# UPM-ROB-Lab/Vision-basedSensor

Measured on AMD Instinct MI355X. Metric: frames/sec (track->3D) at 1280x1024, 169 markers, higher is better.
Workload: dtype u8+f64; 1 GPU; BASELINE config 3/4: 4096 synthetic 1280x1024 gray uint8 frames per GPU (13x13 dots, seeded jitter+noise), resident in HBM; fused track->3D table + last-seen displacement; frames_per_gpu=4096, internal_batch=1536, pass_streams=2, markers=169, channels=1, world_size=1, backend=none (single process), distinct_devices=1, tracked_observations=692224, xyz_solved=692224, ncc_ambiguous_pixels=205, ncc_exact_pixels=11244250, ncc_counter_frames=839680

## Files before the change

vision-basedsensor_amd/csrc/k_ncc_mfma.hip:

```cpp
#include <algorithm>
#include <cstddef>
#include <cstring>
#include <type_traits>

#include "ncc_common.h"

typedef _Float16 h8 __attribute__((ext_vector_type(8)));
typedef _Float16 h4 __attribute__((ext_vector_type(4)));
typedef float f4 __attribute__((ext_vector_type(4)));
typedef float f2 __attribute__((ext_vector_type(2)));
typedef int i4 __attribute__((ext_vector_type(4)));
typedef __attribute__((address_space(1))) u8 gl_u8;
typedef __attribute__((address_space(1))) unsigned short gl_u16;

template <int L> struct NccLit;
template <> struct NccLit<80> { static constexpr float kc = 163.84f, ks2 = 547.2815085234848f, K1 = 3502601.654550303f; };
template <> struct NccLit<33> { static constexpr float kc = 962.8797061524332f, ks2 = 6956.564407359948f, K1 = 7575698.639614983f; };

struct NccKArgs {
    const u64* bits; const double* rx; const double* ry; const uint4* wfrag; const double* tab; const float2* rowf;
    u64* mbits; u8* mask_u8; u32* fstat; u64* tot;
    int H, W, WW, tiles_per_seg, dbg_arg; float rel_arg;
    NccConst nc;
};
typedef __attribute__((address_space(4))) const NccKArgs NccKArgsC;
__device__ __forceinline__ NccKArgsC* ncc_kargs() {
    NccKArgsC* p = (NccKArgsC*)__builtin_amdgcn_kernarg_segment_ptr();
    asm volatile("" : "+s"(p));
    return p;
}

template <int L, int LO, bool U8OUT>
__global__ __launch_bounds__(256, 4) void k_ncc_mfma(const u64* __restrict__ bits, const double* __restrict__ rx,
                                                     const double* __restrict__ ry, const uint4* __restrict__ wfrag,
                                                     const double* __restrict__ tab, const float2* __restrict__ rowf,
                                                     u64* __restrict__ mbits, u8* __restrict__ mask_u8,
                                                     u32* __restrict__ fstat, u64* __restrict__ tot, int H, int W, int WW,
                                                     int tiles_per_seg,
                                                     int dbg_arg, float rel_arg, NccConst nc) {
#ifdef VBS_DEBUG_KNOBS
    const int dbg = dbg_arg & (NCC_TRIM_BIT - 1);
#else
    constexpr int dbg = 0;
#endif
    constexpr int HI = L - 1 + LO;
    constexpr int NT = (16 + L - 1 + 15) / 16;
    constexpr int NKS = (16 * NT + 31) / 32;
    constexpr int NK8 = (16 * NT + 63) / 64;
    constexpr int RING = 16 * NT;
    constexpr int RSTR = RING + 8;
    constexpr int CSTR = RING + 16;
    constexpr int ECAP = 2 * NT + 2;
    __shared__ struct __align__(16) {
        uint4 lut[256];
        _Float16 ring[4][2][16 * RSTR];
        u8 ringc[4][16 * CSTR];
        u32 elist[4][ECAP][10];
    } sm;
    const int tid = threadIdx.x, lane = tid & 63;
    const int wave = __builtin_amdgcn_readfirstlane(tid >> 6);
    const int g = lane >> 4, q = lane & 15;
    const int n = blockIdx.z;
    const int tilesY = (H + 15) / 16;
    const int tile0 = blockIdx.y * tiles_per_seg;
    int ntiles = min(tiles_per_seg, tilesY - tile0);
    if (ntiles <= 0) return;
    int Y0 = tile0 * 16;
    const int xw = blockIdx.x * 64 + 16 * wave;
    const u64* fbits = bits + (int64_t)n * H * WW;
    {
        u32 w[4];
#pragma unroll
        for (int d = 0; d < 4; ++d) w[d] = (((u32)tid >> (2 * d)) & 1u ? 0x3C00u : 0u) | (((u32)tid >> (2 * d + 1)) & 1u ? 0x3C000000u : 0u);
        sm.lut[tid] = make_uint4(w[0], w[1], w[2], w[3]);
    }
    if (dbg_arg & NCC_TRIM_BIT) {
        const int seg_y0 = Y0, seg_y1 = min(Y0 + 16 * ntiles, H);
        const int r0 = max(Y0 + LO, 0), r1 = min(Y0 + 16 * ntiles - 1 + HI, H - 1);
        const int pws = xw + LO, pb0 = pws >> 3;
        const bool pwide = (pb0 >= 0) && ((pb0 & ~3) + 16 <= 8 * WW);
        constexpr int NB = 16 + L - 1;
        int first = 0x7FFFFFFF, last = -1;
        for (int base = r0; base <= r1; base += 256) {
            u64 w0[4], w1[4];
#pragma unroll
            for (int k = 0; k < 4; ++k) {
                const int row = min(base + 64 * k + lane, r1);
                if (pwide) {
                    const uint4 rr = *reinterpret_cast<const uint4*>(reinterpret_cast<const u8*>(fbits) + (pb0 & ~3) + (int64_t)row * (8 * WW));
                    const u64 lo64 = (u64)rr.x | ((u64)rr.y << 32), hi64 = (u64)rr.z | ((u64)rr.w << 32);
                    const int sh = 8 * (pb0 & 3);
                    w0[k] = sh ? (lo64 >> sh) | (hi64 << (64 - sh)) : lo64;
                    w1[k] = hi64 >> sh;
                } else {
                    const u64* prow = fbits + (int64_t)row * WW;
                    w0[k] = load_bits(prow, WW, pws);
                    w1[k] = NB > 64 ? load_bits(prow, WW, pws + 64) : 0ull;
                }
            }
#pragma unroll
            for (int k = 0; k < 4; ++k) {
                const u64 v0 = NB >= 64 ? w0[k] : w0[k] & ((1ull << (NB & 63)) - 1ull);
                const u64 v1 = NB > 64 ? w1[k] & ((1ull << ((NB - 64) & 63)) - 1ull) : 0ull;
                const u64 occ = __ballot((v0 | v1) != 0ull);
                if (occ) {
                    first = min(first, min(base + 64 * k + (int)__builtin_ctzll(occ), r1));
                    last = max(last, min(base + 64 * k + 63 - (int)__builtin_clzll(occ), r1));
                }
            }
        }
        int ta = tile0;
        if (last >= 0) {
            const int tb = min(Y0 + 16 * ntiles - 1, last - LO) >> 4;
            ta = max(Y0, first - HI) >> 4;
            ntiles = tb - ta + 1;
        } else {
            ntiles = 0;
        }
        Y0 = 16 * __builtin_amdgcn_readfirstlane(ta);
        ntiles = __builtin_amdgcn_readfirstlane(ntiles);
        u8* zb = reinterpret_cast<u8*>(reinterpret_cast<unsigned short*>(mbits) + ((int64_t)n * H * WW + blockIdx.x) * 4 + wave);
        for (int y = seg_y0 + lane; y < seg_y1; y += 64)
            if (y < Y0 || y >= Y0 + 16 * ntiles) *reinterpret_cast<unsigned short*>(zb + (int64_t)y * (8 * WW)) = 0;
        if (U8OUT) {
            for (int y = seg_y0 + g; y < seg_y1; y += 4)
                if ((y < Y0 || y >= Y0 + 16 * ntiles) && xw + q < W) mask_u8[((int64_t)n * H + y) * W + xw + q] = 0;
        }
    }
    const int nsteps = ntiles > 0 ? ntiles + NT - 1 : 0;
    h8 whi[NKS], wlo[NKS], one[NKS];
    i4 one8[NK8];
    if (nsteps) {
        for (int i = lane; i < 2 * 16 * RSTR / 8; i += 64) reinterpret_cast<uint4*>(&sm.ring[wave][0][0])[i] = make_uint4(0, 0, 0, 0);
        for (int i = lane; i < 16 * CSTR / 16; i += 64) reinterpret_cast<uint4*>(&sm.ringc[wave][0])[i] = make_uint4(0, 0, 0, 0);
#pragma unroll
        for (int s = 0; s < NKS; ++s) {
            uint4 a = wfrag[(0 * NKS + s) * 64 + lane], b = wfrag[(1 * NKS + s) * 64 + lane], c = wfrag[(2 * NKS + s) * 64 + lane];
            whi[s] = __builtin_bit_cast(h8, a);
            wlo[s] = __builtin_bit_cast(h8, b);
            one[s] = __builtin_bit_cast(h8, c);
        }
#pragma unroll
        for (int s = 0; s < NK8; ++s) {
            const uint4 a = wfrag[(3 * NKS + s) * 64 + lane];
            one8[s] = i4{(int)a.x, (int)a.y, (int)a.z, (int)a.w};
        }
    }
    __builtin_amdgcn_s_waitcnt(0x0F70);
    __syncthreads();

    const double mu = (double)(255ull * (u64)fstat[n * 8 + 0]) / (double)((int64_t)H * W);
    const double full_t = ry[min(max(-LO, 0), H - 1)] * rx[min(max(-LO, 0), W - 1)];
    auto uni = [](float v) { float o; asm("s_nop 4\n\tv_readfirstlane_b32 %0, %1\n\ts_nop 4" : "=s"(o) : "v"(v)); return o; };
    const float kc = uni((float)(nc.tbar * (NCC_WSCALE * NCC_WSCALE)));
    const float th0 = (float)ncc_theta(0.0, nc.l2, full_t, mu, nc);
    bool lit_ok;
    {
        const double ksd = sqrt(nc.thr2 * nc.T2) / (double)L * (NCC_WSCALE * NCC_WSCALE);
        const double k0d = mu * (full_t - nc.l2 * nc.tbar) / 255.0 * (NCC_WSCALE * NCC_WSCALE);
        lit_ok = fabs(nc.tbar * (NCC_WSCALE * NCC_WSCALE) - (double)NccLit<L>::kc) <= 2e-7 * (double)NccLit<L>::kc &&
                 fabs(ksd * ksd - (double)NccLit<L>::ks2) <= 2e-7 * (double)NccLit<L>::ks2 && fabs(k0d) < 1e-4;
    }
    const bool th0pos = __builtin_amdgcn_readfirstlane((th0 > 0.0f && lit_ok) ? 1 : 0) != 0;
    const bool xin = (xw + LO >= 0) && (xw + 15 + HI <= W - 1);
#ifdef VBS_DEBUG_KNOBS
    const int plain_lo = dbg == 10 ? -0x40000000 : (th0pos && xin && dbg != 11) ? -LO : 0x7FFFFFFF, plain_hi = dbg == 10 ? 0x40000000 : H - 1 - 15 - HI;
#else
    const int plain_lo = (th0pos && xin) ? -LO : 0x7FFFFFFF, plain_hi = H - 1 - 15 - HI;
#endif
    const int valid_hi = (xw + 15 < W) ? H - 16 : -1;
    const float muf = uni((float)mu), tbarf = uni((float)nc.tbar), ktf = uni((float)(nc.tbar * 255.0)), il2f = uni((float)nc.inv_l2);
    const float krf = uni((float)(nc.thr2 * nc.T2));
    const float mukf = uni((float)(mu / 255.0 * (NCC_WSCALE * NCC_WSCALE)));
    const int xq = min(xw + q, W - 1);
    const float nxf = (float)(min(xq + HI, W - 1) - max(xq + LO, 0) + 1), rxf = (float)rx[xq];
    const float nnc = (float)L * nxf, stc = (float)ry[min(max(-LO, 0), H - 1)] * rxf, dd0c = stc - nnc * tbarf;
    _Float16* const ringw = &sm.ring[wave][0][q * RSTR];
    _Float16* const wr = ringw + 4 * g;
    const _Float16* const rd = ringw + 8 * g;
    const _Float16* const rdw = rd - (g >= 2 ? RING : 0);
    u8* const cw = &sm.ringc[wave][q * CSTR] + 4 * g;
    const u8* const cbase = &sm.ringc[wave][q * CSTR];
    constexpr int LOFS = 16 * RSTR;
    u32 amb = 0, nexact = 0;
    unsigned short* mb16 = reinterpret_cast<unsigned short*>(mbits) + ((int64_t)n * H * WW + blockIdx.x) * 4 + wave;
    const int wstart = xw + LO;
    static_assert((LO & 7) == 0, "the window must start on a byte of the row");
    const int rowbytes = 8 * WW, b0 = wstart >> 3;
    int wide_i = __builtin_amdgcn_readfirstlane(((b0 >= 0) && ((b0 & ~3) + 16 <= rowbytes)) ? 1 : 0);
    asm volatile("" : "+s"(wide_i));
#define wide (wide_i != 0)
    uint4 nraw = make_uint4(0, 0, 0, 0);
    const u8* fby = reinterpret_cast<const u8*>(fbits) + (b0 & ~3);
    const u32 lofs = (u32)(q * rowbytes);
    const u32 psel = 0x0C0C0C00u | (u32)((b0 & 3) + g);
    auto load_rows = [&](int t) {
        const int ytile = Y0 + LO + 16 * t;
        if (wide) {
            const gl_u8* pg;
            if (ytile >= 0 && ytile + 15 < H) {
                const u8* pb = fby + (int64_t)ytile * rowbytes;
                asm volatile("" : "+s"(pb));
                u32 lo_ = lofs;
                asm volatile("" : "+v"(lo_));
                pg = (const gl_u8*)pb + lo_;
            } else {
                pg = (const gl_u8*)fby + (u32)__mul24(min(max(ytile + q, 0), H - 1), rowbytes);
            }
            typedef u32 u32x4 __attribute__((ext_vector_type(4)));
            typedef __attribute__((address_space(1))) const u32x4 gl_u4;
            const u32x4 rr = *(gl_u4*)pg;
            nraw = make_uint4(rr.x, rr.y, rr.z, rr.w);
        } else {
            const u64* row = fbits + (int64_t)min(max(ytile + q, 0), H - 1) * WW;
            int ws = __builtin_amdgcn_readfirstlane(wstart);
            asm volatile("" : "+s"(ws));
            const u64 w0 = load_bits(row, WW, ws), w1 = NKS > 2 ? load_bits(row, WW, ws + 64) : 0ull;
            const u32 dw[4] = {(u32)w0, (u32)(w0 >> 32), (u32)w1, (u32)(w1 >> 32)};
            const u32 sh = 8 * (b0 & 3);
            nraw = make_uint4(dw[0] << sh, sh ? __builtin_amdgcn_alignbit(dw[1], dw[0], 32 - sh) : dw[1],
                              sh ? __builtin_amdgcn_alignbit(dw[2], dw[1], 32 - sh) : dw[2],
                              sh ? __builtin_amdgcn_alignbit(dw[3], dw[2], 32 - sh) : dw[3]);
        }
    };
    int ecnt = 0;
    constexpr int NO_TILE = 0x7FFFFFFF;
    u32 pend_x = 0;
    int pend_yo = NO_TILE;
    const u32 off_lo = (u32)((8 * (lane & 1) + ((lane >> 1) & 3)) * rowbytes), off_hi = off_lo + (u32)(4 * rowbytes);
    auto flush_pending = [&]() {
        if (pend_yo != NO_TILE) {
            u8* base = reinterpret_cast<u8*>(mb16) + (int64_t)pend_yo * rowbytes;
            asm volatile("" : "+s"(base));
            gl_u8* bg = (gl_u8*)base;
            u32 ol_ = off_lo, oh_ = off_hi;
            asm volatile("" : "+v"(ol_), "+v"(oh_));
            if (pend_yo <= H - 16) {
                if (lane < 8) {
                    *(gl_u16*)(bg + ol_) = (unsigned short)pend_x;
                    *(gl_u16*)(bg + oh_) = (unsigned short)(pend_x >> 16);
                }
            } else {
                const int rl = pend_yo + 8 * (lane & 1) + ((lane >> 1) & 3);
                if (lane < 8 && rl < H) *(gl_u16*)(bg + ol_) = (unsigned short)pend_x;
                if (lane < 8 && rl + 4 < H) *(gl_u16*)(bg + oh_) = (unsigned short)(pend_x >> 16);
            }
        }
        pend_yo = NO_TILE;
    };
    auto drain = [&]() {
        __builtin_amdgcn_s_waitcnt(0x0F70);
        constexpr bool RELOAD = L < 64;
        const double *d_tab, *d_rx, *d_ry; u64* d_mbits; u8* d_mask_u8; int d_H, d_W, d_WW;
        double d_nc_tbar, d_nc_inv_l2, d_nc_thr2, d_nc_T2, d_mu; const u64* d_fbits;
        if constexpr (RELOAD) {
            NccKArgsC* ka = ncc_kargs();
            d_tab = ka->tab; d_rx = ka->rx; d_ry = ka->ry; d_mbits = ka->mbits; d_mask_u8 = ka->mask_u8;
            d_H = ka->H; d_W = ka->W; d_WW = ka->WW;
            d_nc_tbar = ka->nc.tbar; d_nc_inv_l2 = ka->nc.inv_l2; d_nc_thr2 = ka->nc.thr2; d_nc_T2 = ka->nc.T2;
            d_mu = (double)(255ull * (u64)ka->fstat[n * 8 + 0]) / (double)((int64_t)d_H * d_W);
            d_fbits = ka->bits + (int64_t)n * d_H * d_WW;
        } else {
            d_tab = tab; d_rx = rx; d_ry = ry; d_mbits = mbits; d_mask_u8 = mask_u8; d_H = H; d_W = W; d_WW = WW;
            d_nc_tbar = nc.tbar; d_nc_inv_l2 = nc.inv_l2; d_nc_thr2 = nc.thr2; d_nc_T2 = nc.T2; d_mu = mu; d_fbits = fbits;
        }
        const double* cgd = d_tab + VBS_NCC_MAXL;
        u32* mb32 = reinterpret_cast<u32*>(d_mbits) + (int64_t)n * d_H * d_WW * 2;
        for (int e = 0; e < ecnt; ++e) {
            const int yo = (int)__builtin_amdgcn_readfirstlane((int)sm.elist[wave][e][0]);
#pragma unroll 1
            for (int r = 0; r < 4; ++r) {
                u64 ur = (u64)(u32)__builtin_amdgcn_readfirstlane((int)sm.elist[wave][e][2 + 2 * r]) |
                         ((u64)(u32)__builtin_amdgcn_readfirstlane((int)sm.elist[wave][e][3 + 2 * r]) << 32);
                while (ur) {
                    const int l = __ffsll((long long)ur) - 1;
                    ur &= ur - 1ull;
                    const int y = yo + 4 * (l >> 4) + r, xe = xw + (l & 15);
                    double hv[(L + 63) / 64];
                    u32 cnt = 0;
#pragma unroll
                    for (int k = 0; k < (L + 63) / 64; ++k) {
                        const int i = lane + 64 * k, yy = y + LO + i;
                        hv[k] = (i < L && yy >= 0 && yy < d_H) ? ncc_row_exact<L, LO>(d_fbits + (int64_t)yy * d_WW, d_WW, xe, cgd, &cnt) : 0.0;
                    }
#pragma unroll
                    for (int off = 32; off >= 1; off >>= 1) cnt += (u32)__shfl_xor((int)cnt, off);
                    double Ge = 0.0;
#pragma unroll
                    for (int k = 0; k < (L + 63) / 64; ++k) {
                        const u32 hl = (u32)__double_as_longlong(hv[k]), hh = (u32)((u64)__double_as_longlong(hv[k]) >> 32);
#pragma unroll 8
                        for (int i = 64 * k; i < min(L, 64 * k + 64); ++i) {
                            const u64 hb = (u64)(u32)__builtin_amdgcn_readlane((int)hl, i - 64 * k) |
                                           ((u64)(u32)__builtin_amdgcn_readlane((int)hh, i - 64 * k) << 32);
                            Ge = __builtin_fma(d_tab[i], __longlong_as_double((long long)hb), Ge);
                        }
                    }
                    int ny = min(y + HI, d_H - 1) - max(y + LO, 0) + 1;
                    int nx = min(xe + HI, d_W - 1) - max(xe + LO, 0) + 1;
                    double nn = (double)(ny * nx), sum_t = d_ry[y] * d_rx[xe];
                    double sum_I = 255.0 * (double)cnt;
                    double rest = -d_nc_tbar * sum_I - d_mu * (sum_t - nn * d_nc_tbar);
                    double s1 = sum_I - nn * d_mu;
                    double s2 = 255.0 * sum_I - 2.0 * d_mu * sum_I + nn * d_mu * d_mu;
                    double var = s2 - s1 * s1 * d_nc_inv_l2;
                    double rhs = d_nc_thr2 * var * d_nc_T2;
                    double num = 255.0 * Ge + rest;
                    const int flags = __builtin_amdgcn_readfirstlane((var > 0.0 ? 1 : 0) | ((var > 0.0 && num > 0.0 && num * num > rhs) ? 2 : 0) |
                                                                     ((var > 1e-6 && num > 0.0 && fabs(num * num - rhs) <= 1e-9 * rhs) ? 4 : 0));
                    if ((flags & 2) && lane == 0) {
                        atomicOr(&mb32[(u32)__mul24(y, 2 * d_WW) + (u32)(xe >> 5)], 1u << (xe & 31));
                        if (U8OUT) d_mask_u8[((int64_t)n * d_H + y) * d_W + xe] = 1;
                    }
                    if (flags & 1) { nexact++; if (flags & 4) amb++; }
                }
            }
        }
        ecnt = 0;
    };
    h8 a_op[NKS];
    auto fetch_ops = [&](int tt) {
        u32 by[NKS];
        const u32 rw[5] = {nraw.x, nraw.y, nraw.z, nraw.w, 0u};
#pragma unroll
        for (int s = 0; s < NKS; ++s) by[s] = __builtin_amdgcn_perm(rw[s + 1], rw[s], psel);
#pragma unroll
        for (int s = 0; s < NKS; ++s) asm volatile("" : "+v"(by[s]) :: "memory");
        load_rows(tt + 1);
        flush_pending();
        const int ytile = Y0 + LO + 16 * tt;
        if (ytile < 0 || ytile + 15 >= H) {
            const bool rowin = (ytile + q >= 0) && (ytile + q < H);
#pragma unroll
            for (int s = 0; s < NKS; ++s) by[s] = rowin ? by[s] : 0u;
        }
#pragma unroll
        for (int s = 0; s < NKS; ++s) a_op[s] = __builtin_bit_cast(h8, sm.lut[by[s]]);
    };
    if (nsteps) {
        load_rows(0);
        fetch_ops(0);
    }
    for (int t0 = 0; t0 < nsteps; t0 += NT) {
#pragma unroll
        for (int u = 0; u < NT; ++u) {
            const int t = t0 + u;
            if (t >= nsteps) break;
            constexpr int dummy_nt = NT;
            const int B = (u + 1) % dummy_nt;
            constexpr int NKE = (RING - 16) / 32;
            constexpr int NK8E = (RING - 16) / 64;
            f4 G = {0, 0, 0, 0};
            i4 C = {0, 0, 0, 0};
            auto vert_f16 = [&](int s) {
                const int r0 = (16 * B + 32 * s) % RING;
                const _Float16* p = (r0 + 32 <= RING ? rd : rdw) + r0;
                const h8 bh = *reinterpret_cast<const h8*>(p);
                const h8 bl = *reinterpret_cast<const h8*>(p + LOFS);
                G = __builtin_amdgcn_mfma_f32_16x16x32_f16(whi[s], bh, G, 0, 0, 0);
                G = __builtin_amdgcn_mfma_f32_16x16x32_f16(whi[s], bl, G, 0, 0, 0);
                G = __builtin_amdgcn_mfma_f32_16x16x32_f16(wlo[s], bh, G, 0, 0, 0);
            };
            auto vert_i8 = [&](int s) {
                const int gi = min(4 * s + g, NT - 1);
                const int slot = B + gi - (gi >= NT - B ? NT : 0);
                const i4 bc = *reinterpret_cast<const i4*>(cbase + 16 * slot);
                C = __builtin_amdgcn_mfma_i32_16x16x64_i8(one8[s], bc, C, 0, 0, 0);
            };
            const bool vert = !(t < NT - 1 || dbg == 3);
            f4 ah = {0, 0, 0, 0}, ac = {0, 0, 0, 0};
            if (vert) {
#pragma unroll
                for (int s = 0; s < NKS; ++s) {
                    ah = __builtin_amdgcn_mfma_f32_16x16x32_f16(a_op[s], whi[s], ah, 0, 0, 0);
                    if (s < NKE) vert_f16(s);
                    ah = __builtin_amdgcn_mfma_f32_16x16x32_f16(a_op[s], wlo[s], ah, 0, 0, 0);
                    if (s < NK8E) vert_i8(s);
                    ac = __builtin_amdgcn_mfma_f32_16x16x32_f16(a_op[s], one[s], ac, 0, 0, 0);
                }
#pragma unroll
                for (int s = NKS; s < NKE; ++s) vert_f16(s);
            } else {
#pragma unroll
                for (int s = 0; s < NKS; ++s) {
                    ah = __builtin_amdgcn_mfma_f32_16x16x32_f16(a_op[s], whi[s], ah, 0, 0, 0);
                    ah = __builtin_amdgcn_mfma_f32_16x16x32_f16(a_op[s], wlo[s], ah, 0, 0, 0);
                    ac = __builtin_amdgcn_mfma_f32_16x16x32_f16(a_op[s], one[s], ac, 0, 0, 0);
                }
            }
            fetch_ops(t + 1);
            {
                h4 vh, vl;
#pragma unroll
                for (int r = 0; r < 4; ++r) {
                    const float hi_f = __uint_as_float(__float_as_uint(ah[r]) & 0xFFFFE000u);
                    vh[r] = (_Float16)hi_f;
                    vl[r] = (_Float16)(ah[r] - hi_f);
                }
                u32 vc = 0;
#pragma unroll
                for (int r = 0; r < 4; ++r) vc = __builtin_amdgcn_cvt_pk_u8_f32(ac[r], r, vc);
                *reinterpret_cast<h4*>(wr + 16 * u) = vh;
                *reinterpret_cast<h4*>(wr + LOFS + 16 * u) = vl;
                *reinterpret_cast<u32*>(cw + 16 * u) = vc;
            }
            if (!vert) continue;
            const int yo = Y0 + 16 * (t - (NT - 1));
#pragma unroll
            for (int s = NKE; s < NKS; ++s) vert_f16(s);
#pragma unroll
            for (int s = NK8E; s < NK8; ++s) vert_i8(s);
#ifdef VBS_DEBUG_KNOBS
            if (dbg == 8 && mask_u8) {
#pragma unroll
                for (int r = 0; r < 4; ++r) {
                    const int y = yo + 4 * g + r, x = xw + q;
                    if (y < H && x < W) mask_u8[((int64_t)n * H + y) * W + x] = (u8)C[r];
                }
                continue;
            }
#endif
            if (dbg == 2) { asm volatile("" :: "v"(G[0]), "v"(G[1]), "v"(G[2]), "v"(G[3]), "v"(C[0]), "v"(C[1]), "v"(C[2]), "v"(C[3])); continue; }
            const int x = xw + q;
            float cf[4];
#pragma unroll
            for (int r = 0; r < 4; ++r) cf[r] = (float)C[r];
            u64 pw[4] = {0, 0, 0, 0}, uw[4] = {0, 0, 0, 0};
            if (yo >= plain_lo && yo <= plain_hi) {
                const float rel = rel_arg;
                float uu[4], uhi[4];
#pragma unroll
                for (int r = 0; r < 4; ++r) {
                    uu[r] = __builtin_fmaf(cf[r], -NccLit<L>::kc, G[r]);
                    uhi[r] = __builtin_fmaf(G[r], rel, uu[r]);
                }
                const float umax = fmaxf(fmaxf(uhi[0], uhi[1]), fmaxf(uhi[2], uhi[3]));
                if (__ballot(umax >= 0.0f) || dbg == 12) {
#pragma unroll
                    for (int r = 0; r < 4; ++r) {
                        const float ulo = __builtin_fmaf(G[r], -rel, uu[r]);
                        const float a = __builtin_fmaf(cf[r], -NccLit<L>::ks2, NccLit<L>::K1) * cf[r];
                        pw[r] = __ballot(ulo * fabsf(ulo) > a);
                        uw[r] = ~(pw[r] | __ballot(uhi[r] * fabsf(uhi[r]) <= a));
                    }
                }
            } else {
                float nnv[4], stv[4], dd0[4], uhi[4];
                if (yo + LO >= 0 && yo <= plain_hi) {
#pragma unroll
                    for (int r = 0; r < 4; ++r) { nnv[r] = nnc; stv[r] = stc; dd0[r] = dd0c; }
                } else {
#pragma unroll
                    for (int r = 0; r < 4; ++r) {
                        const float2 rf = rowf[min(yo + 4 * g + r, H - 1)];
                        nnv[r] = rf.x * nxf;
                        stv[r] = rf.y * rxf;
                        dd0[r] = stv[r] - nnv[r] * tbarf;
                    }
                }
#pragma unroll
                for (int r = 0; r < 4; ++r) {
                    const float kcc = kc * cf[r];
                    const float mrg = __builtin_fmaf(1e-3f, G[r] + kcc, __builtin_fmaf(1e-5f * mukf, stv[r], 2.0f));
                    uhi[r] = (G[r] - kcc) - mukf * dd0[r] + mrg;
                }
                if (__ballot(fmaxf(fmaxf(uhi[0], uhi[1]), fmaxf(uhi[2], uhi[3])) >= 0.0f)) {
#pragma unroll
                    for (int r = 0; r < 4; ++r) {
                        const float cfr = cf[r];
                        const float nn = nnv[r], a0 = 1.0f - nn * il2f;
                        const float rest = -(ktf * cfr) - muf * dd0[r];
                        const float var = 65025.0f * cfr * (1.0f - cfr * il2f) + a0 * muf * (nn * muf - 510.0f * cfr);
                        const float t1 = (__builtin_amdgcn_sqrtf(fmaxf(krf * var, 0.0f)) - rest) * (float)(NCC_WSCALE * NCC_WSCALE / 255.0);
                        const float t0v = ((dd0[r] > -1e-4f) | (dd0[r] * dd0[r] < 0.5f * krf * a0 * nn)) ? (float)NCC_NEVER : 0.0f;
                        const float th = cfr == 0.0f ? t0v : t1;
                        const float m = __builtin_fmaf(fabsf(th), 1e-3f, 2.0f), d = G[r] - th;
                        pw[r] = __ballot(d > m);
                        uw[r] = ~(pw[r] | __ballot(d < -m));
                    }
                }
            }
            if (yo > valid_hi) {
#pragma unroll
                for (int r = 0; r < 4; ++r) {
                    const u64 v = __ballot((yo + 4 * g + r < H) && (x < W));
                    pw[r] &= v; uw[r] &= v;
                }
            }
#ifdef VBS_DEBUG_KNOBS
            if (dbg == 9 && mask_u8) {
#pragma unroll
                for (int r = 0; r < 4; ++r) {
                    const int y = yo + 4 * g + r;
                    if (y < H && x < W) mask_u8[((int64_t)n * H + y) * W + x] = (u8)(((pw[r] >> lane) & 1ull) | (((uw[r] >> lane) & 1ull) << 1));
                }
                continue;
            }
#endif
            if (uw[0] | uw[1] | uw[2] | uw[3]) {
                if (lane == 0) {
                    u32* e = &sm.elist[wave][ecnt][0];
                    e[0] = (u32)yo;
#pragma unroll
                    for (int r = 0; r < 4; ++r) { e[2 + 2 * r] = (u32)uw[r]; e[3 + 2 * r] = (u32)(uw[r] >> 32); }
                }
                ecnt++;
            }
            if (U8OUT) {
#pragma unroll
                for (int r = 0; r < 4; ++r) {
                    const int y = yo + 4 * g + r;
                    if (y < H && x < W) mask_u8[((int64_t)n * H + y) * W + x] = (u8)((pw[r] >> lane) & 1ull);
                }
            }
            if (dbg == 1) { asm volatile("" :: "s"(pw[0]), "s"(pw[1]), "s"(pw[2]), "s"(pw[3])); continue; }
            {
                u32 xv = 0;
#pragma unroll
                for (int r = 0; r < 4; ++r) {
                    asm("v_writelane_b32 %0, %1, %2" : "+v"(xv) : "s"((u32)pw[r]), "n"(2 * r));
                    asm("v_writelane_b32 %0, %1, %2" : "+v"(xv) : "s"((u32)(pw[r] >> 32)), "n"(2 * r + 1));
                }
                pend_x = xv;
                pend_yo = yo;
            }
        }
        if (t0 + NT >= nsteps || ecnt > ECAP - NT) {
            flush_pending();
            if (ecnt) drain();
        }
    }
    {
        u32* fstat_ = fstat; u64* tot_ = tot;
        if constexpr (L < 64) { NccKArgsC* ka = ncc_kargs(); fstat_ = ka->fstat; tot_ = ka->tot; }
        if (lane == 0) {
            if (amb) { atomicAdd(&fstat_[n * 8 + 1], amb); atomicAdd(&tot_[0], (u64)amb); }
            if (nexact) { atomicAdd(&fstat_[n * 8 + 3], nexact); atomicAdd(&tot_[1], (u64)nexact); }
        }
        if (tid == 0 && (blockIdx.x | blockIdx.y | blockIdx.z) == 0) atomicAdd(&tot_[2], (u64)gridDim.z);
    }
}
#undef wide

using NccKernelFn = void (*)(decltype(NccKArgs::bits), decltype(NccKArgs::rx), decltype(NccKArgs::ry), decltype(NccKArgs::wfrag),
                             decltype(NccKArgs::tab), decltype(NccKArgs::rowf), decltype(NccKArgs::mbits), decltype(NccKArgs::mask_u8),
                             decltype(NccKArgs::fstat), decltype(NccKArgs::tot), decltype(NccKArgs::H), decltype(NccKArgs::W),
                             decltype(NccKArgs::WW), decltype(NccKArgs::tiles_per_seg), decltype(NccKArgs::dbg_arg),
                             decltype(NccKArgs::rel_arg), decltype(NccKArgs::nc));
static_assert(std::is_same_v<decltype(&k_ncc_mfma<80, -40, true>), NccKernelFn> && std::is_same_v<decltype(&k_ncc_mfma<80, -40, false>), NccKernelFn> &&
              std::is_same_v<decltype(&k_ncc_mfma<33, -16, true>), NccKernelFn> && std::is_same_v<decltype(&k_ncc_mfma<33, -16, false>), NccKernelFn>,
              "NccKArgs does not mirror k_ncc_mfma's parameter list");
static_assert(std::is_standard_layout_v<NccKArgs> && offsetof(NccKArgs, nc) == 104 && alignof(NccConst) == 8,
              "NccKArgs does not lay out as the kernarg segment does");

std::vector<u32> ncc_mfma_fragments(const NccConst& nc, int l) {
    const int nt = (16 + l - 1 + 15) / 16, nks = (16 * nt + 31) / 32, nk8 = (16 * nt + 63) / 64;
    std::vector<u32> out((size_t)(3 * nks + nk8) * 64 * 4, 0);
    for (int s = 0; s < nk8; ++s)
        for (int lane = 0; lane < 64; ++lane)
            for (int j = 0; j < 16; ++j) {
                const int idx = 64 * s + 16 * (lane >> 4) + j - (lane & 15);
                if (idx >= 0 && idx < l) out[((size_t)(3 * nks + s) * 64 + lane) * 4 + (j >> 2)] |= 1u << (8 * (j & 3));
            }
    auto bits16 = [](double v) { _Float16 hv = (_Float16)v; unsigned short b; memcpy(&b, &hv, 2); return (u32)b; };
    for (int kind = 0; kind < 3; ++kind)
        for (int s = 0; s < nks; ++s)
            for (int lane = 0; lane < 64; ++lane) {
                const int g = lane >> 4, col = lane & 15;
                for (int j = 0; j < 8; ++j) {
                    const int idx = 32 * s + 8 * g + j - col;
                    u32 v = 0;
                    if (idx >= 0 && idx < l) {
                        const double w = nc.g[idx] * NCC_WSCALE;
                        const _Float16 hi = (_Float16)w;
                        v = kind == 0 ? bits16((double)hi) : kind == 1 ? bits16(w - (double)hi) : bits16(1.0);
                    }
                    out[((size_t)(kind * nks + s) * 64 + lane) * 4 + (j >> 1)] |= v << (16 * (j & 1));
                }
            }
    return out;
}

void launch_ncc_mfma(vbs_handle* h, Workspace& w, int nb, u8* mask_u8, hipStream_t s) {
    const int tilesY = (h->H + 15) / 16;
    const int want = h->WW * nb <= 512 ? 1024 : 2048;
    int nseg = std::min(tilesY, std::max(1, want == 1024 ? want / (h->WW * nb) : (want + h->WW * nb - 1) / (h->WW * nb)));
    if (VBS_KNOB("VBS_NCC_NSEG")) nseg = VBS_KNOB("VBS_NCC_NSEG");
    const int tps = (tilesY + nseg - 1) / nseg;
    nseg = (tilesY + tps - 1) / tps;
    dim3 grid(h->WW, nseg, nb);
    const int trim = (h->ncc_trim_ok && !VBS_KNOB("VBS_NCC_DBG") && !VBS_KNOB("VBS_NCC_TRIM_OFF")) ? NCC_TRIM_BIT : 0;
#define NCC_GO(L_, LO_, U8)                                                                                      \
    VBS_LAUNCH(h, s, "k_ncc_mfma", (k_ncc_mfma<L_, LO_, U8>), grid, dim3(256), 0, s, w.area_bits, h->ncc_rx,     \
               h->ncc_ry, h->ncc_frags, h->ncc_tab, h->ncc_rowf, w.mask_bits, mask_u8, w.fstat, w.ncc_tot,       \
               h->H, h->W, h->WW, tps,                                                                           \
               VBS_KNOB("VBS_NCC_DBG") | trim, std::max(NCC_REL, 1e-6f * (float)h->ncc_margin_ppm), h->ncc)
    if (!h->bp.small) { if (mask_u8) NCC_GO(80, -40, true); else NCC_GO(80, -40, false); }
    else { if (mask_u8) NCC_GO(33, -16, true); else NCC_GO(33, -16, false); }
#undef NCC_GO
}
```

vision-basedsensor_amd/csrc/ncc_common.h:

```cpp
#pragma once
#include "common.h"

__device__ __forceinline__ u64 load_bits(const u64* __restrict__ row, int WW, int start) {
    int wi = start >> 6, sh = start & 63;
    u64 a = (wi >= 0 && wi < WW) ? row[wi] : 0ull;
    u64 b = (wi + 1 >= 0 && wi + 1 < WW) ? row[wi + 1] : 0ull;
    return sh ? ((a >> sh) | (b << (64 - sh))) : a;
}

template <int L, int LO>
__device__ __forceinline__ double ncc_row_exact(const u64* __restrict__ row, int WW, int x, const double* cg,
                                                u32* cnt) {
    u64 w0 = load_bits(row, WW, x + LO), w1 = 0;
    if (L > 64) w1 = load_bits(row, WW, x + LO + 64) & ((1ull << (L > 64 ? L - 64 : 1)) - 1ull);
    else w0 &= (1ull << (L < 64 ? L : 0)) - 1ull;
    *cnt += __popcll(w0) + __popcll(w1);
    double h = 0.0;
#pragma unroll
    for (int half = 0; half < 2; ++half) {
        u64 w = half ? w1 : w0;
        while (w) {
            int b0 = __ffsll((long long)w) - 1;
            u64 t = ~(w >> b0);
            int len = t ? __ffsll((long long)t) - 1 : 64 - b0;
            w &= (len >= 64) ? 0ull : ~(((1ull << len) - 1ull) << b0);
            h += cg[half * 64 + b0 + len] - cg[half * 64 + b0];
        }
    }
    return h;
}

template <int L, int LO>
__device__ __attribute__((noinline)) double ncc_exact_G(const u64* fbits, int H, int WW, int y, int x, const double* cg,
                                                        const double* gsh) {
    u32 dummy = 0;
    double Ge = 0.0;
    for (int i = 0; i < L; ++i) {
        int yy = y + LO + i;
        double hrow = (yy >= 0 && yy < H) ? ncc_row_exact<L, LO>(fbits + (int64_t)yy * WW, WW, x, cg, &dummy) : 0.0;
        Ge = __builtin_fma(gsh[i], hrow, Ge);
    }
    return Ge;
}

#define NCC_WSCALE 1024.0
#define NCC_REL 2e-5f
#define NCC_NEVER 3e38
#define NCC_TRIM_BIT 0x100
#define NCC_ABS 1e-3f

__device__ __forceinline__ double ncc_theta(double c, double nn, double sum_t, double mu, const NccConst& nc) {
    double sum_I = 255.0 * c;
    double rest = -nc.tbar * sum_I - mu * (sum_t - nn * nc.tbar);
    double s1 = sum_I - nn * mu;
    double s2 = 255.0 * sum_I - 2.0 * mu * sum_I + nn * mu * mu;
    double var = s2 - s1 * s1 * nc.inv_l2;
    double rhs = nc.thr2 * var * nc.T2;
    if (!(var > 0.0)) return NCC_NEVER;
    if (c == 0.0) return (rest > 0.0 && rest * rest > rhs) ? -NCC_NEVER : NCC_NEVER;
    return (sqrt(rhs) - rest) * (NCC_WSCALE * NCC_WSCALE / 255.0);
}
```

Before: 315,100 frames/s.

## Share row-occupancy scan across block waves and skip empty pipeline ramp steps

Reworks the NCC trim prescan so each thread loads three adjacent bit-words per row for 256 rows at once, and each wave computes occupancy ranges for all four sub-windows. The results are shared through shared memory, which replaces four redundant per-wave scans with one cooperative scan. It also computes a kskip so the MFMA pipeline starts at the first tile whose window touches occupied rows, skipping empty ramp-up steps. Blocks with no work now exit early after a counter update. This adds a __syncthreads and extra register pressure in the prescan, and the early-exit path changes how the counter is accounted.

```diff
diff --git a/vision-basedsensor_amd/csrc/k_ncc_mfma.hip b/vision-basedsensor_amd/csrc/k_ncc_mfma.hip
--- a/vision-basedsensor_amd/csrc/k_ncc_mfma.hip
+++ b/vision-basedsensor_amd/csrc/k_ncc_mfma.hip
@@ -74,51 +74,80 @@
         for (int d = 0; d < 4; ++d) w[d] = (((u32)tid >> (2 * d)) & 1u ? 0x3C00u : 0u) | (((u32)tid >> (2 * d + 1)) & 1u ? 0x3C000000u : 0u);
         sm.lut[tid] = make_uint4(w[0], w[1], w[2], w[3]);
     }
-    if (dbg_arg & NCC_TRIM_BIT) {
-        const int seg_y0 = Y0, seg_y1 = min(Y0 + 16 * ntiles, H);
+    int kskip = 0;
+    const bool trim = (dbg_arg & NCC_TRIM_BIT) != 0;
+    const int seg_y0 = Y0, seg_y1 = min(Y0 + 16 * ntiles, H);
+    if (trim) {
         const int r0 = max(Y0 + LO, 0), r1 = min(Y0 + 16 * ntiles - 1 + HI, H - 1);
-        const int pws = xw + LO, pb0 = pws >> 3;
-        const bool pwide = (pb0 >= 0) && ((pb0 & ~3) + 16 <= 8 * WW);
         constexpr int NB = 16 + L - 1;
+        constexpr int PR = 5;
+        const int wl = (int)blockIdx.x - 1;
+        const bool in0 = wl >= 0, in2 = wl + 2 < WW;
+        int pfirst[4], plast[4];
+#pragma unroll
+        for (int s = 0; s < 4; ++s) { pfirst[s] = 0x7FFFFFFF; plast[s] = -1; }
+        for (int base = r0; base <= r1; base += 256 * PR) {
+            u64 a[PR][3];
+#pragma unroll
+            for (int j = 0; j < PR; ++j) {
+                const int rb = base + 256 * j;
+                const u64* prow = fbits + (int64_t)min(rb + tid, r1) * WW + wl;
+                a[j][0] = (in0 && rb <= r1) ? prow[0] : 0ull;
+                a[j][1] = rb <= r1 ? prow[1] : 0ull;
+                a[j][2] = (in2 && rb <= r1) ? prow[2] : 0ull;
+            }
+#pragma unroll
+            for (int j = 0; j < PR; ++j) {
+                const int rw = base + 256 * j + 64 * wave;
+                if (rw > r1) break;
+                const bool rin = rw + lane <= r1;
+#pragma unroll
+                for (int s = 0; s < 4; ++s) {
+                    const int sb = 64 + 16 * s + LO, se = sb + NB;
+                    u64 v = 0ull;
+#pragma unroll
+                    for (int i = 0; i < 3; ++i) {
+                        const int lo_ = max(sb, 64 * i) - 64 * i, hi_ = min(se, 64 * i + 64) - 64 * i;
+                        if (hi_ > lo_) v |= a[j][i] & ((hi_ - lo_ >= 64 ? ~0ull : ((1ull << ((hi_ - lo_) & 63)) - 1ull)) << lo_);
+                    }
+                    const u64 occ = __ballot(rin && v != 0ull);
+                    if (occ) {
+                        pfirst[s] = min(pfirst[s], rw + (int)__builtin_ctzll(occ));
+                        plast[s] = max(plast[s], rw + 63 - (int)__builtin_clzll(occ));
+                    }
+                }
+            }
+        }
+        if (lane == 0) {
+#pragma unroll
+            for (int s = 0; s < 4; ++s) { sm.elist[wave][0][2 * s] = (u32)pfirst[s]; sm.elist[wave][0][2 * s + 1] = (u32)plast[s]; }
+        }
+    }
+    __syncthreads();
+    if (trim) {
         int first = 0x7FFFFFFF, last = -1;
-        for (int base = r0; base <= r1; base += 256) {
-            u64 w0[4], w1[4];
-#pragma unroll
-            for (int k = 0; k < 4; ++k) {
-                const int row = min(base + 64 * k + lane, r1);
-                if (pwide) {
-                    const uint4 rr = *reinterpret_cast<const uint4*>(reinterpret_cast<const u8*>(fbits) + (pb0 & ~3) + (int64_t)row * (8 * WW));
-                    const u64 lo64 = (u64)rr.x | ((u64)rr.y << 32), hi64 = (u64)rr.z | ((u64)rr.w << 32);
-                    const int sh = 8 * (pb0 & 3);
-                    w0[k] = sh ? (lo64 >> sh) | (hi64 << (64 - sh)) : lo64;
-                    w1[k] = hi64 >> sh;
-                } else {
-                    const u64* prow = fbits + (int64_t)row * WW;
-                    w0[k] = load_bits(prow, WW, pws);
-                    w1[k] = NB > 64 ? load_bits(prow, WW, pws + 64) : 0ull;
-                }
-            }
-#pragma unroll
-            for (int k = 0; k < 4; ++k) {
-                const u64 v0 = NB >= 64 ? w0[k] : w0[k] & ((1ull << (NB & 63)) - 1ull);
-                const u64 v1 = NB > 64 ? w1[k] & ((1ull << ((NB - 64) & 63)) - 1ull) : 0ull;
-                const u64 occ = __ballot((v0 | v1) != 0ull);
-                if (occ) {
-                    first = min(first, min(base + 64 * k + (int)__builtin_ctzll(occ), r1));
-                    last = max(last, min(base + 64 * k + 63 - (int)__builtin_clzll(occ), r1));
-                }
-            }
-        }
+#pragma unroll
+        for (int v = 0; v < 4; ++v) {
+            first = min(first, (int)sm.elist[v][0][2 * wave]);
+            last = max(last, (int)sm.elist[v][0][2 * wave + 1]);
+        }
+        first = __builtin_amdgcn_readfirstlane(first);
+        last = __builtin_amdgcn_readfirstlane(last);
         int ta = tile0;
         if (last >= 0) {
             const int tb = min(Y0 + 16 * ntiles - 1, last - LO) >> 4;
             ta = max(Y0, first - HI) >> 4;
             ntiles = tb - ta + 1;
+            kskip = min((first - (16 * ta + LO)) >> 4, NT - 1);
         } else {
             ntiles = 0;
         }
+#ifdef VBS_DEBUG_KNOBS
+        if (dbg_arg & NCC_RAMP_OFF_BIT) kskip = 0;
+#endif
         Y0 = 16 * __builtin_amdgcn_readfirstlane(ta);
         ntiles = __builtin_amdgcn_readfirstlane(ntiles);
+        kskip = __builtin_amdgcn_readfirstlane(kskip);
         u8* zb = reinterpret_cast<u8*>(reinterpret_cast<unsigned short*>(mbits) + ((int64_t)n * H * WW + blockIdx.x) * 4 + wave);
         for (int y = seg_y0 + lane; y < seg_y1; y += 64)
             if (y < Y0 || y >= Y0 + 16 * ntiles) *reinterpret_cast<unsigned short*>(zb + (int64_t)y * (8 * WW)) = 0;
@@ -148,6 +177,10 @@
     }
     __builtin_amdgcn_s_waitcnt(0x0F70);
     __syncthreads();
+    if (!nsteps) {
+        if (tid == 0 && (blockIdx.x | blockIdx.y | blockIdx.z) == 0) atomicAdd(&tot[2], (u64)gridDim.z);
+        return;
+    }
 
     const double mu = (double)(255ull * (u64)fstat[n * 8 + 0]) / (double)((int64_t)H * W);
     const double full_t = ry[min(max(-LO, 0), H - 1)] * rx[min(max(-LO, 0), W - 1)];
@@ -338,13 +371,14 @@
         for (int s = 0; s < NKS; ++s) a_op[s] = __builtin_bit_cast(h8, sm.lut[by[s]]);
     };
     if (nsteps) {
-        load_rows(0);
-        fetch_ops(0);
+        load_rows(kskip);
+        fetch_ops(kskip);
     }
     for (int t0 = 0; t0 < nsteps; t0 += NT) {
 #pragma unroll
         for (int u = 0; u < NT; ++u) {
             const int t = t0 + u;
+            if (t < kskip) continue;
             if (t >= nsteps) break;
             constexpr int dummy_nt = NT;
             const int B = (u + 1) % dummy_nt;
@@ -589,7 +623,8 @@
     const int tps = (tilesY + nseg - 1) / nseg;
     nseg = (tilesY + tps - 1) / tps;
     dim3 grid(h->WW, nseg, nb);
-    const int trim = (h->ncc_trim_ok && !VBS_KNOB("VBS_NCC_DBG") && !VBS_KNOB("VBS_NCC_TRIM_OFF")) ? NCC_TRIM_BIT : 0;
+    const int trim = (h->ncc_trim_ok && !VBS_KNOB("VBS_NCC_DBG") && !VBS_KNOB("VBS_NCC_TRIM_OFF"))
+                         ? NCC_TRIM_BIT | (VBS_KNOB("VBS_NCC_RAMP_OFF") ? NCC_RAMP_OFF_BIT : 0) : 0;
 #define NCC_GO(L_, LO_, U8)                                                                                      \
     VBS_LAUNCH(h, s, "k_ncc_mfma", (k_ncc_mfma<L_, LO_, U8>), grid, dim3(256), 0, s, w.area_bits, h->ncc_rx,     \
                h->ncc_ry, h->ncc_frags, h->ncc_tab, h->ncc_rowf, w.mask_bits, mask_u8, w.fstat, w.ncc_tot,       \
diff --git a/vision-basedsensor_amd/csrc/ncc_common.h b/vision-basedsensor_amd/csrc/ncc_common.h
--- a/vision-basedsensor_amd/csrc/ncc_common.h
+++ b/vision-basedsensor_amd/csrc/ncc_common.h
@@ -47,6 +47,7 @@
 #define NCC_REL 2e-5f
 #define NCC_NEVER 3e38
 #define NCC_TRIM_BIT 0x100
+#define NCC_RAMP_OFF_BIT 0x200
 #define NCC_ABS 1e-3f
 
 __device__ __forceinline__ double ncc_theta(double c, double nn, double sum_t, double mu, const NccConst& nc) {
```

New measurement: 317,500 frames/s (median of 6 runs). No clear change (+0.8%).
